# terran-project/terran

Hardware: AMD Instinct MI355X
Metric: frames/sec 1080p detect+embed+pose (higher is better)
Workload: dtype f16x3: operands x = hi + lo (two IEEE halfs, 22 bits), 3 f16 MFMAs per product, f32 accumulate; float32-grade results; 1 GPU; BASELINE configs[4]: 1080p detect+embed+pose; Detection(short_side=416) + Recognition(top-2) + Estimation(short_side=184); 32 frames per GPU per step resident in HBM; random-init weights; precision=f16x3, frames_per_gpu_step=32, faces_per_frame=2, resident_batch_reused=True, batches_in_flight_per_gpu=2

## Files before the change

### terran_amd/build.py

```python
import os
import subprocess
import sys

HERE = os.path.dirname(os.path.abspath(__file__))
CSRC = os.path.join(HERE, 'csrc')
LIB = os.path.join(HERE, 'libterran_amd.so')
SOURCES = ['runtime.hip', 'conv_split.hip', 'conv_split_modes.hip', 'conv_sym.hip', 'conv_dwpw.hip', 'conv_igemm.hip', 'layers.hip', 'net.hip', 'retinaface_post.hip', 'arcface_post.hip',
           'openpose_post.hip', 'draw.hip', 'jpeg_host.hip', 'jpeg.hip',
           'jpeg_encode.hip']
FLAGS = ['--offload-arch=gfx950', '-O3', '-std=c++17', '-fPIC', '-Wall', '-Wno-unused-function']


STAMP = LIB + '.stamp'


def source_hash():
    import hashlib
    h = hashlib.sha256(' '.join(FLAGS).encode())
    files = [os.path.join(CSRC, f) for f in sorted(os.listdir(CSRC)) if f.endswith(('.hip', '.h'))]
    files.append(os.path.join(os.path.dirname(HERE), 'include', 'terran_amd.h'))
    for f in files:
        with open(f, 'rb') as fh:
            h.update(os.path.basename(f).encode() + b'\0' + fh.read())
    return h.hexdigest()


def _stale(target, deps):
    if not os.path.exists(target):
        return True
    t = os.path.getmtime(target)
    return any(os.path.getmtime(d) > t for d in deps)


def _unit_hash(src, headers, flags):
    import hashlib
    h = hashlib.sha256(' '.join(flags).encode())
    for f in [src] + sorted(headers):
        with open(f, 'rb') as fh:
            h.update(os.path.basename(f).encode() + b'\0' + fh.read())
    return h.hexdigest()


def build(force=False, verbose=False):
    hipcc = os.environ.get('HIPCC', '/opt/rocm/bin/hipcc')
    headers = [os.path.join(CSRC, f) for f in os.listdir(CSRC) if f.endswith('.h')]
    headers.append(os.path.join(os.path.dirname(HERE), 'include', 'terran_amd.h'))
    extra_all = os.environ.get('TA_EXTRA_FLAGS', '').split()
    objs = []
    procs = []
    for src in SOURCES:
        s = os.path.join(CSRC, src)
        if not os.path.exists(s):
            continue
        o = os.path.join(CSRC, src.replace('.hip', '.o'))
        objs.append(o)
        exact = src.endswith('_post.hip') or src == 'draw.hip'
        flags = FLAGS + (['-ffp-contract=off'] if exact else []) + extra_all
        want = _unit_hash(s, headers, flags)
        try:
            with open(o + '.stamp') as fh:
# ... 88 lines not shown
```

### terran_amd/csrc/net.hip

```cpp
#include <stdlib.h>
#include <string.h>

#include <algorithm>
#include <chrono>

#include "act_format.h"
#include "ta_internal.h"

static int conv_out(int in, int k, int stride, int pad) { return (in + 2 * pad - k) / stride + 1; }

static bool conv_ksplit_eligible(const ta_op_desc& op, int in_fmt) {
  const int kblk = in_fmt == TA_FMT_F16 ? 64 : 32;
  const bool uniform = (op.cin % kblk == 0) && (op.n_slabs == op.kh * op.kw * (op.cin / kblk));
  const bool kernel_ok = in_fmt == ta_split_fmt_of(op.prec);
  return uniform && kernel_ok && op.groups <= 1 && !op.pool;
}

#define TA_MAX_PLANS 4
#define TA_MAX_PLAN_BYTES ((size_t)96 << 30)

static void destroy_plan(ta_plan* pl) {
  if (!pl) return;
  if (pl->arena) (void)hipFree(pl->arena);
  if (pl->ktab_dev) (void)hipFree(pl->ktab_dev);
// ... 232 lines not shown
static const float* wptr(const ta_model* m, int64_t off) { return off < 0 ? nullptr : (const float*)(m->weights_dev + off); }

static void print_op_profile(ta_model* m, std::vector<hipEvent_t>& ev) {
  (void)hipStreamSynchronize(m->ctx->stream);
  double tot_ms = 0, tot_fl = 0;
  for (size_t oi = 0; oi < m->ops.size(); ++oi) {
    const ta_op_desc& op = m->ops[oi];
    const ta_tensor& to = m->tensors[op.out];
    float ms = 0.f;
    (void)hipEventElapsedTime(&ms, ev[2 * oi], ev[2 * oi + 1]);
    const ta_tensor& ti = m->tensors[op.in];
    const double M = op.type == TA_OP_CONV && op.pool
                         ? (double)m->run_n * conv_out(ti.h, op.kh, op.stride, op.pad) * conv_out(ti.w, op.kw, op.stride, op.pad)
                         : (double)m->run_n * to.h * to.w;
    const double fl = (op.type == TA_OP_CONV || op.type == TA_OP_DWPW) ? 2.0 * op.macs_per_pixel * M : 0.0;
    tot_ms += ms;
    tot_fl += fl;
    fprintf(stderr, "op %3zu type %d k%dx%d s%d g%d cin %4d cout %4d  %3dx%-3d M %8.0f slabs %4d  %8.1f us %7.1f TF\n", oi, op.type, op.kh,
            op.kw, op.stride, op.groups, op.cin, op.cout, to.h, to.w, M, op.n_slabs, ms * 1e3, ms > 0 ? fl / (ms * 1e-3) / 1e12 : 0.0);
  }
  fprintf(stderr, "model kind %d n %d: %.3f ms in ops, %.1f GFLOP, %.1f TF\n", m->kind, m->run_n, tot_ms, tot_fl / 1e9, tot_fl / (tot_ms * 1e-3) / 1e12);
  for (auto e : ev) (void)hipEventDestroy(e);
}

int ta_model_run_ops(ta_model* m) {
  ta_ctx* ctx = m->ctx;
  static const bool prof_ops = getenv("TA_PROFILE_OPS") != nullptr;
  std::vector<hipEvent_t> ev;
  if (prof_ops) {
    ev.resize(2 * m->ops.size());
    for (auto& e : ev) (void)hipEventCreate(&e);
  }
  struct fin_t {
    ta_model* m;
    std::vector<hipEvent_t>& ev;
    bool on;
    ~fin_t() { if (on) print_op_profile(m, ev); }
  } fin{m, ev, prof_ops};
  static const bool no_lanes = getenv("TA_NO_LANES") != nullptr;
  const bool lanes_on = !prof_ops && !ctx->profiling && !no_lanes;
  struct lanes_t {
    ta_ctx* ctx;
    hipStream_t main;
    bool started[2] = {false, false};
    ~lanes_t() {
      ctx->stream = main;
      for (int i = 0; i < 2; ++i)
        if (started[i]) {
          (void)hipEventRecord(ctx->side_join[i], ctx->side_stream[i]);
          (void)hipStreamWaitEvent(main, ctx->side_join[i], 0);
        }
    }
  } lanes{ctx, ctx->stream};
  for (size_t oi = 0; oi < m->ops.size(); ++oi) {
    const ta_op_desc& op = m->ops[oi];
    const ta_tensor& ti = m->tensors[op.in];
    const ta_tensor& to = m->tensors[op.out];
    const int lane = lanes_on ? (op.variant >> 17) & 3 : 0;
    ctx->stream = lanes.main;
    if (lane) {
      const int li = lane - 1;
      if (!ctx->side_stream[li]) {
        TA_HIP(ctx, hipStreamCreateWithFlags(&ctx->side_stream[li], hipStreamNonBlocking));
        TA_HIP(ctx, hipEventCreateWithFlags(&ctx->side_fork[li], hipEventDisableTiming));
        TA_HIP(ctx, hipEventCreateWithFlags(&ctx->side_join[li], hipEventDisableTiming));
      }
      if (!lanes.started[li]) {
        TA_HIP(ctx, hipEventRecord(ctx->side_fork[li], lanes.main));
        TA_HIP(ctx, hipStreamWaitEvent(ctx->side_stream[li], ctx->side_fork[li], 0));
        lanes.started[li] = true;
      }
      ctx->stream = ctx->side_stream[li];
    }
    struct evp_t {
      hipEvent_t e;
      hipStream_t s;
      bool on;
      ~evp_t() { if (on) (void)hipEventRecord(e, s); }
    } evp{prof_ops ? ev[2 * oi + 1] : nullptr, ctx->stream, prof_ops};
    if (prof_ops) (void)hipEventRecord(ev[2 * oi], ctx->stream);
    switch (op.type) {
      case TA_OP_CONV: {
        ta_conv_launch p;
        memset(&p, 0, sizeof(p));
        p.in = ti.dev;
        p.w = wptr(m, op.w_off);
        p.ktab = m->ktab_dev + m->ktab_off[oi];
        p.bias = wptr(m, op.bias_off);
        p.prelu = wptr(m, op.prelu_off);
        p.out = to.dev;
        p.M = m->run_n * to.h * to.w;
        p.Ho = to.h;
        p.Wo = to.w;
        p.n_slabs = op.n_slabs;
        p.coutp = op.coutp;
        p.cout = op.cout;
        p.act = op.act;
        p.stride = op.stride;
        p.prec = op.prec;
        const int kblk = ti.fmt == TA_FMT_F16 ? 64 : 32;
        p.uniform_k = (op.cin % kblk == 0) && (op.n_slabs == op.kh * op.kw * (op.cin / kblk));
        p.k_cblocks = op.cin / kblk;
        if (ti.fmt == TA_FMT_F16 && (!p.uniform_k || op.in_ch_off || op.groups > 1 || op.prec != 4))
          return ta_fail(ctx, TA_E_INVALID, "op %zu: a half-float tensor feeds whole-tensor convs of the f16 mode only", oi);
        p.k_w = op.kw;
        p.k_h = op.kh;
// ... 2 lines not shown
        p.in_row = ti.wp() * ti.cf();
        p.in_pix = ti.cf();
        p.win_wp = ti.wp();
        p.win_img = ti.hp() * ti.wp();
        p.in_off0 = (int)(((size_t)(ti.halo - op.pad) * ti.wp() + (ti.halo - op.pad)) * ti.cf());
        p.out_img = (int)((size_t)to.hp() * to.wp() * to.cf());
        p.out_row = to.wp() * to.cf();
        p.out_pix = to.cf();
        p.out_off0 = (int)to.off(0, 0, 0);
        p.out_ch = op.out_ch_off;
        p.out_fmt = to.fmt;
        p.in_fmt = ti.fmt;
        if (op.res >= 0) {
          const ta_tensor& tr = m->tensors[op.res];
          p.res = tr.dev;
          p.res_img = (int)((size_t)tr.hp() * tr.wp() * tr.cf());
          p.res_row = tr.wp() * tr.cf();
          p.res_pix = tr.cf();
          p.res_off0 = (int)tr.off(0, 0, 0);
          p.res_ch = op.res_ch_off;
          p.res_fmt = tr.fmt;
          p.res_up2 = op.res_up2;
        }
        if (op.out2 >= 0) {
          const ta_tensor& t2 = m->tensors[op.out2];
          p.out2 = t2.dev;
          p.scale2 = wptr(m, op.scale2_off);
          p.shift2 = wptr(m, op.shift2_off);
          p.o2_img = (int)((size_t)t2.hp() * t2.wp() * t2.cf());
          p.o2_row = t2.wp() * t2.cf();
          p.o2_pix = t2.cf();
          p.o2_off0 = (int)t2.off(0, 0, 0);
          p.o2_ch = op.out2_ch_off;
          p.o2_fmt = t2.fmt;
        }
        if (op.groups > 1) {
          p.group_cout = op.cout / op.groups;
          p.group_cin = op.cin;
        }
        p.variant = op.variant & 255;
        if ((op.variant >> 16) & 1) p.bias9 = wptr(m, op.scale2_off);
        p.range_check = (m->has_half_ops && (m->tensor_read[op.out] || (op.out2 >= 0 && m->tensor_read[op.out2]))) ? 1 : 0;
        p.amax_index = (m->amax_on && oi < TA_AMAX_OPS) ? (int)oi : -1;
        double flops = 2.0 * op.macs_per_pixel * (double)p.M;
        if (op.pool) {
          p.pool = 1;
          p.M = m->run_n * to.h * to.w * 4;
          flops = 2.0 * op.macs_per_pixel * (double)m->run_n * conv_out(ti.h, op.kh, op.stride, op.pad) *
                  conv_out(ti.w, op.kw, op.stride, op.pad);
        }
        p.k_split = m->splitk_ws ? ta_conv_ksplit(p.coutp, p.n_slabs, conv_ksplit_eligible(op, ti.fmt), (op.variant >> 8) & 255) : 1;
        p.partial = m->splitk_ws;
        if (lane) p.k_split = 1;
        TA_TRY(ta_launch_conv(ctx, p, flops));
        break;
      }
      case TA_OP_RFSTEM:
        TA_TRY(ta_launch_rfstem(ctx, m->input_u8, m->run_n, ti.h, ti.w, (const float*)m->weights_host_small.data(),
                                op.cout == 32 ? wptr(m, op.w_off) + 448 : nullptr, to));
        break;
      case TA_OP_DWPW: {
        ta_conv_launch p;
        memset(&p, 0, sizeof(p));
        p.in = ti.dev;
        p.w = wptr(m, op.w_off);
        p.bias = wptr(m, op.bias_off);
        p.dw_w = wptr(m, op.scale2_off);
        p.dw_bias = wptr(m, op.shift2_off);
        p.dw_c = op.cin;
        p.dw_stride = op.stride;
        p.out = to.dev;
        p.M = m->run_n * to.h * to.w;
        p.Ho = to.h;
        p.Wo = to.w;
        p.n_slabs = op.n_slabs;
        p.coutp = op.coutp;
        p.cout = op.cout;
        p.act = op.act;
        p.stride = 1;
        p.prec = op.prec;
        p.range_check = (m->has_half_ops && m->tensor_read[op.out]) ? 1 : 0;
        p.amax_index = (m->amax_on && oi < TA_AMAX_OPS) ? (int)oi : -1;
        p.in_img = (int)((size_t)ti.hp() * ti.wp() * ti.c);
        p.in_row = ti.wp() * ti.c;
        p.in_pix = ti.c;
        p.in_off0 = (int)(((size_t)(ti.halo - 1) * ti.wp() + (ti.halo - 1)) * ti.c);
        p.in_fmt = ti.fmt;
        p.out_img = (int)((size_t)to.hp() * to.wp() * to.c);
        p.out_row = to.wp() * to.c;
        p.out_pix = to.c;
        p.out_off0 = (int)to.off(0, 0, 0);
        p.out_ch = op.out_ch_off;
        p.out_fmt = to.fmt;
        TA_TRY(ta_launch_dwpw(ctx, p, 2.0 * op.macs_per_pixel * (double)p.M));
        break;
      }
      case TA_OP_DWCONV: {
        ta_dw_launch p;
        memset(&p, 0, sizeof(p));
        p.in = ti.dev;
        p.w = wptr(m, op.w_off);
        p.bias = wptr(m, op.bias_off);
        p.out = to.dev;
        p.N = m->run_n;
        p.Ho = to.h;
        p.Wo = to.w;
// ... 349 lines not shown
```

### terran_amd/csrc/ta_internal.h

```cpp
#pragma once
#include <hip/hip_runtime.h>
#include <stdint.h>
#include <stdio.h>
#include <atomic>
#include <map>
#include <mutex>
#include <string>
#include <vector>

#include "../../include/terran_amd.h"

#define TA_BLOB_MAGIC 0x314D4154u

enum {
  TA_OP_CONV = 1,
  TA_OP_DWCONV = 2,
  TA_OP_MAXPOOL = 3,
  TA_OP_COPYCH = 4,
  TA_OP_RFSTEM = 5,
  TA_OP_DWPW = 6
};
enum { TA_ACT_NONE = 0, TA_ACT_RELU = 1, TA_ACT_PRELU = 2 };

struct ta_blob_header {
// ... 201 lines not shown
struct ta_conv_launch {
  const float* in;
  const float* w;
  const int32_t* ktab;
  const float* bias;
  const float* prelu;
  float* out;
  const float* res;
  float* out2;
  const float* scale2;
  const float* shift2;
  int M, Ho, Wo, n_slabs, coutp, cout, act, stride, prec;
  int uniform_k, k_cblocks, k_w, k_h, in_ch_off;
  int in_img, in_row, in_pix, in_off0;
  int out_img, out_row, out_pix, out_off0, out_ch, out_fmt;
  int res_img, res_row, res_pix, res_off0, res_up2, res_ch, res_fmt;
  int o2_img, o2_row, o2_pix, o2_off0, o2_ch, o2_fmt;
  int in_fmt;
  int win_wp, win_img;
  int group_cout, group_cin;
  int k_split;
  float* partial;
  int variant;
  const float* dw_w;
  const float* dw_bias;
  int dw_c, dw_stride;
  int pool;
  float r_nct, r_tile_blocks, r_Wo, r_Ho, r_HoWo;
  int fast_div;
  int fast_drain;
#ifdef TA_CONV_TRACE
  int trace_block;
#endif
  const float* bias9;
  int range_check;
  int amax_index;
  int* range_flag;
};

static inline int ta_split_fmt_of(int prec) { return prec == 0 ? 0  : (prec == 4 ? 3  : ((prec == 3 || prec == 5) ? 2  : 1 )); }

static inline int ta_conv_ksplit(int coutp, int n_slabs, bool eligible, int packed = 0) {
  if (!eligible || coutp % 128) return 1;
  if (packed > 1) return packed <= n_slabs ? packed : 1;
  if (n_slabs < 512) return 1;
  return 32;
}

int ta_launch_conv(ta_ctx* ctx, const ta_conv_launch& p, double flops);
int ta_launch_conv_sym(ta_ctx* ctx, int variant, const ta_conv_launch& p);
int ta_launch_conv_split(ta_ctx* ctx, int variant, const ta_conv_launch& p);
int ta_launch_conv_split_modes(ta_ctx* ctx, int variant, const ta_conv_launch& p);
int ta_launch_dwpw(ta_ctx* ctx, const ta_conv_launch& p, double flops);
int ta_win_patch_rows(const ta_conv_launch& p, int BM);
#define TA_WIN_PR_2x2 384
#define TA_WIN_PR_2x4 448
#define TA_WIN_PR_1x4 512
struct ta_frames;
int ta_launch_rfstem(ta_ctx* ctx, const uint8_t* frames_dev, int n, int h, int w, const float* weights_host, const float* w2_dev, const struct ta_tensor& out);

struct ta_dw_launch {
  const float* in;
  const float* w;
  const float* bias;
  float* out;
  int N, Ho, Wo, C, stride, relu;
  int in_img, in_row, in_pix, in_off0, in_fmt;
  int out_img, out_row, out_pix, out_off0, out_fmt;
};
int ta_launch_dwconv(ta_ctx* ctx, const ta_dw_launch& p);
int ta_launch_maxpool(ta_ctx* ctx, const ta_tensor& in, const ta_tensor& out, int n);
int ta_launch_copych(ta_ctx* ctx, const ta_tensor& in, int in_ch, const ta_tensor& out, int out_ch, int ch, int n);

enum { TA_PRE_RETINAFACE = 1, TA_PRE_OPENPOSE = 2, TA_PRE_ARCFACE_CROPS = 3 };
int ta_launch_preprocess(ta_ctx* ctx, int mode, const uint8_t* src_dev, int n, int h, int w, const ta_tensor& dst);

struct ta_plan {
  int n = 0, h = 0, w = 0;
  std::vector<ta_tensor> tensors;
  char* arena = nullptr;
  size_t arena_bytes = 0;
  int32_t* ktab_dev = nullptr;
  std::vector<size_t> ktab_off;
  float* splitk_ws = nullptr;
  uint64_t last_use = 0;
};

struct ta_model {
  ta_ctx* ctx = nullptr;
  int kind = 0;
  ta_blob_header hdr;
  std::vector<ta_tensor_desc> tdesc;
  std::vector<ta_op_desc> ops;
  char* weights_dev = nullptr;
  bool has_half_ops = false;
  bool amax_on = false;
  std::vector<char> tensor_read;
  std::vector<std::vector<float>> unscale_host;
  std::vector<char> weights_host_small;
  std::vector<ta_plan*> plans;
  ta_plan* active = nullptr;
  uint64_t use_counter = 0;
  int plan_n = 0, plan_h = 0, plan_w = 0;
  int run_n = 0;
  const uint8_t* input_u8 = nullptr;
  std::vector<ta_tensor> tensors;
// ... 8 lines not shown
```

### terran_amd/pack.py

```python
import os

import numpy as np

from . import arch

MODEL_RETINAFACE, MODEL_ARCFACE, MODEL_OPENPOSE = 1, 2, 3
OP_CONV, OP_DWCONV, OP_MAXPOOL, OP_COPYCH, OP_RFSTEM, OP_DWPW = 1, 2, 3, 4, 5, 6
ACT_NONE, ACT_RELU, ACT_PRELU = 0, 1, 2
MAGIC = 0x314D4154

HEADER_DT = np.dtype({
    'names': ['magic', 'version', 'kind', 'n_tensors', 'n_ops', 'input_tensor', 'n_outputs', 'outputs',
              'tensors_off', 'ops_off', 'weights_off', 'weights_bytes'],
    'formats': ['<u4', '<u4', '<i4', '<i4', '<i4', '<i4', '<i4', ('<i4', 16), '<i8', '<i8', '<i8', '<i8'],
    'offsets': [0, 4, 8, 12, 16, 20, 24, 28, 96, 104, 112, 120],
    'itemsize': 128,
})
TENSOR_DT = np.dtype([('channels', '<i4'), ('halo', '<i4'), ('alias_of', '<i4'), ('fmt', '<i4'), ('unscale_off', '<i4')])
FMT_F32, FMT_SPLIT, FMT_SPLIT16, FMT_F16 = 0, 1, 2, 3
_OP_I32 = ['type', 'in', 'out', 'in_ch_off', 'cin', 'out_ch_off', 'cout', 'coutp', 'kh', 'kw', 'stride', 'pad',
           'act', 'res', 'res_ch_off', 'res_up2', 'out2', 'out2_ch_off', 'n_slabs', 'prec', 'groups', 'variant', 'pool', 'wscale_log2']
_OP_I64 = ['w_off', 'bias_off', 'prelu_off', 'scale2_off', 'shift2_off', 'wus_off']
OP_DT = np.dtype([(n, '<i4') for n in _OP_I32] + [(n, '<i8') for n in _OP_I64] + [('macs_per_pixel', '<f8')])
assert OP_DT.itemsize == 152 and TENSOR_DT.itemsize == 20
BLOB_VERSION = 9


PACK_SWITCHES = ('TERRAN_AMD_NO_FUSED_POOL', 'TERRAN_AMD_NO_GROUPED', 'TERRAN_AMD_NO_MERGED_OUTPUTS', 'TERRAN_AMD_ARCFACE_SECOND_OUTPUT',
                 'TERRAN_AMD_NO_STAGE4_KSPLIT', 'TERRAN_AMD_DETECTOR_F32', 'TERRAN_AMD_DETECTOR_BASE_F32', 'TERRAN_AMD_NO_FUSED_DETECTOR', 'TERRAN_AMD_NO_FUSED_FRONT',
                 'TERRAN_AMD_NO_DETECTOR_LANES', 'TERRAN_AMD_NO_ACT_SCALES')


def active_switches():
    return tuple((k, os.environ[k]) for k in PACK_SWITCHES if os.environ.get(k))


_SOURCE_TAG = []


def source_tag():
    if not _SOURCE_TAG:
        import hashlib
        h = hashlib.sha256()
        here = os.path.dirname(os.path.abspath(__file__))
        try:
            for f in ('pack.py', 'arch.py'):
                with open(os.path.join(here, f), 'rb') as fh:
                    h.update(fh.read())
            _SOURCE_TAG.append(h.hexdigest()[:10])
        except OSError:
            _SOURCE_TAG.append(None)
    return _SOURCE_TAG[0]


PRECISIONS = {'f32': 0, 'bf16x3': 1, 'bf16': 2, 'f16x3': 3, 'f16': 4, 'f16x2': 5}
SPLIT_FMT = {0: FMT_F32, 1: FMT_SPLIT, 2: FMT_SPLIT, 3: FMT_SPLIT16, 4: FMT_F16, 5: FMT_SPLIT16}


def _rup(x, m):
    return (x + m - 1) // m * m


def _bf16_bits(x):
    u = np.ascontiguousarray(x, dtype=np.float32).view(np.uint32)
    return ((u + np.uint32(0x7FFF) + ((u >> np.uint32(16)) & np.uint32(1))) >> np.uint32(16)).astype(np.uint16)


def _bf16_to_f32(b):
    return (b.astype(np.uint32) << np.uint32(16)).view(np.float32)


def split_bf16_rows(packed):
    hi = _bf16_bits(packed)
    lo = _bf16_bits(packed - _bf16_to_f32(hi))
    rows = np.concatenate([hi, lo], axis=-1)
    return np.ascontiguousarray(rows).view(np.float32)


def row_exponents(packed):
    m = np.abs(np.asarray(packed, np.float32)).max(axis=(0, 2)).astype(np.float64)
    ok = np.isfinite(m) & (m > 0)
    s = np.zeros(m.shape, np.int64)
    s[ok] = np.clip(13 - np.floor(np.log2(m[ok])), -60, 60).astype(np.int64)
# ... 134 lines not shown
            if tid == self.input_tensor:
                self.stats[tid][2][:] = True
        return self.stats[tid]

    def _write_stats(self, tid, ch_off, mu, var, amax=None):
        st = self._stats_of(tid)
        n = len(mu)
        if amax is None:
            amax = np.abs(mu) + _ACT_SIGMAS * np.sqrt(var)
        new = ~st[2][ch_off:ch_off + n]
        take = new | (amax > st[3][ch_off:ch_off + n])
        st[0][ch_off:ch_off + n][take] = mu[take]
        st[1][ch_off:ch_off + n][take] = var[take]
        st[3][ch_off:ch_off + n] = np.where(new, amax, np.maximum(amax, st[3][ch_off:ch_off + n]))
        st[2][ch_off:ch_off + n] = True

    @staticmethod
    def _act_bound(mu, var, act, slope=None):
        sd = np.sqrt(np.maximum(var, 0.0))
        hi, lo = mu + _ACT_SIGMAS * sd, _ACT_SIGMAS * sd - mu
        if act == ACT_NONE:
            return np.maximum(hi, lo)
        if act == ACT_RELU or slope is None:
            return np.maximum(hi, 4.0 * sd)
        a = np.abs(np.asarray(slope, np.float64))
        return np.maximum(np.maximum(hi, a * lo), 4.0 * sd * np.maximum(a, 1.0))

    @staticmethod
    def _conv_moments(full, bias, mu_in, var_in, groups, cout):
        taps, cin_p, coutp = full.shape
        f64 = full.astype(np.float64)
        wsum = f64.sum(0)
        wsq = (f64 * f64).sum(0)
        rho = _TAP_CORR if taps > 1 else 0.0
        wvar = (1.0 - rho) * wsq + rho * wsum * wsum
        mu = np.zeros(coutp)
        var = np.zeros(coutp)
        if groups > 1:
            cg = cout // groups
            for g in range(groups):
                sl = slice(g * cg, (g + 1) * cg)
                mu[sl] = mu_in[g * cin_p:(g + 1) * cin_p] @ wsum[:, sl]
                var[sl] = var_in[g * cin_p:(g + 1) * cin_p] @ wvar[:, sl]
        else:
            mu = mu_in[:cin_p] @ wsum
            var = var_in[:cin_p] @ wvar
        b = np.zeros(coutp)
        if bias is not None:
            b[:cout] = np.asarray(bias, np.float64)
        return (mu + b)[:cout], np.maximum(var[:cout], 0.0)

    def conv(self, tin, tout, W, bias, *, stride=1, pad=None, act=ACT_NONE, in_ch_off=0, ch_pos=None, cin_p=None,
             out_ch_off=0, cout_p=None, prelu=None, res=-1, res_ch_off=0, res_up2=0, out2=-1, out2_ch_off=0,
             scale2=None, shift2=None, groups=1, variant=0, pool=False, k_split=0, precision=None, in_affine=None):
        W = np.asarray(W, dtype=np.float64)
        cout, cin, kh, kw = W.shape
        bias9 = None
        if in_affine is not None:
            assert (kh, kw, stride) == (3, 3, 1) and pad in (None, 1) and groups == 1 and out2 < 0 and scale2 is None and not pool
            W, bias9 = fold_input_affine(W, bias, *in_affine)
            bias = bias9[5]
        if groups > 1:
            assert cout % groups == 0 and cin % 32 == 0 and (cout // groups) % 128 == 0 and ch_pos is None
        if pad is None:
            pad = kh // 2
        if pool:
            assert groups == 1 and res < 0 and out2 < 0 and stride == 1 and cin % 32 == 0 and cout % 64 == 0 and ch_pos is None
        if cin_p is None:
            cin_p = _rup(cin, 4)
        if ch_pos is None:
            ch_pos = np.arange(cin)
        if cout_p is None:
            cout_p = _rup(cout, 4)
        coutp = _rup(cout_p, 32)
        K = kh * kw * cin_p
        n_slabs = _rup(K, 32) // 32
        full = np.zeros((kh * kw, cin_p, coutp), np.float32)
        full[:, np.asarray(ch_pos), :cout] = W.transpose(2, 3, 1, 0).reshape(kh * kw, cin, cout)
        flat = np.zeros((n_slabs * 32, coutp), np.float32)
        flat[:K] = full.reshape(K, coutp)
        prec = self.prec if precision is None else PRECISIONS[precision]

        def vec(v, fill=0.0):
            if v is None:
                return -1, None
            out = np.full(coutp, fill, np.float64)
            out[:cout] = np.asarray(v, dtype=np.float64)
            return self._w(out), out
        fold = dict(flat=flat, taps=kh * kw, cin_p=cin_p, K=K)
        scale2_off = -1
        if bias9 is not None:
            t9 = np.zeros((16, coutp), np.float64)
            t9[:, :cout] = bias9
            scale2_off = self._w(t9)
            fold['bias9'] = t9
            variant |= 1 << 16
        else:
            scale2_off, fold['scale2'] = vec(scale2)
        bvec = np.zeros(coutp, np.float64)
        if bias is not None:
            bvec[:cout] = np.asarray(bias, np.float64)
        fold['bias'] = bvec
        bias_off = self._w(np.concatenate([bvec, np.ones(coutp)]))
        wus_off = bias_off + 4 * coutp
        prelu_off, _ = vec(prelu)
        shift2_off, fold['shift2'] = vec(shift2)
        op = dict(type=OP_CONV, out=tout, in_ch_off=in_ch_off, cin=cin_p, out_ch_off=out_ch_off, cout=cout_p,
                  coutp=coutp, kh=kh, kw=kw, stride=stride, pad=pad, act=act, res=res, res_ch_off=res_ch_off,
                  res_up2=res_up2, out2=out2, out2_ch_off=out2_ch_off, n_slabs=n_slabs, prec=prec,
                  groups=groups, variant=variant | (int(k_split) << 8) | (self.lane << 17), pool=int(bool(pool)), wscale_log2=0,
                  w_off=self._w_reserve(n_slabs * coutp * 128), bias_off=bias_off, prelu_off=prelu_off, scale2_off=scale2_off,
                  shift2_off=shift2_off, wus_off=wus_off, macs_per_pixel=float(cout * cin * kh * kw))
        op['in'] = tin
        self._fold[len(self.ops)] = fold
        self.ops.append(op)
        st_in = self._stats_of(tin)
        span = cin_p * max(groups, 1)
        mu, var = self._conv_moments(full, bias, st_in[0][in_ch_off:in_ch_off + span], st_in[1][in_ch_off:in_ch_off + span],
                                     groups, cout)
        slope = None if prelu is None else np.asarray(prelu, np.float64)
        bound = self._act_bound(mu, var, act, slope)
        mu, var = act_moments(mu, var, act, slope)
        if res >= 0:
            st_r = self._stats_of(res)
            mu = mu + st_r[0][res_ch_off:res_ch_off + cout]
            var = var + st_r[1][res_ch_off:res_ch_off + cout]
            bound = bound + st_r[3][res_ch_off:res_ch_off + cout]
        if pool:
            mu, var = mu + 1.03 * np.sqrt(var), 0.49 * var
        self._write_stats(tout, out_ch_off, mu, var, bound)
        if out2 >= 0:
            s2, h2 = np.asarray(scale2, np.float64), np.asarray(shift2, np.float64)
            self._write_stats(out2, out2_ch_off, mu * s2 + h2, var * s2 * s2, np.abs(s2) * bound + np.abs(h2))

    def dwconv(self, tin, tout, W, bias, *, stride=1, relu=True):
        C = W.shape[0]
        w9 = np.asarray(W, dtype=np.float64).reshape(C, 9).T
        op = dict(type=OP_DWCONV, out=tout, in_ch_off=0, cin=C, out_ch_off=0, cout=C, coutp=_rup(C, 32), kh=3,
                  kw=3, stride=stride, pad=1, act=ACT_RELU if relu else ACT_NONE, res=-1, res_ch_off=0, res_up2=0,
                  out2=-1, out2_ch_off=0, n_slabs=0, prec=0, groups=1, variant=0, pool=0, wscale_log2=0, w_off=self._w(w9), bias_off=self._w(bias),
                  prelu_off=-1, scale2_off=-1, shift2_off=-1, wus_off=-1, macs_per_pixel=float(C * 9))
        op['in'] = tin
        self.ops.append(op)
        st = self._stats_of(tin)
        mu, var = self._dw_moments(w9, bias, st[0][:C], st[1][:C])
        act = ACT_RELU if relu else ACT_NONE
        self._write_stats(tout, 0, *act_moments(mu, var, act), self._act_bound(mu, var, act))

    @staticmethod
    def _dw_moments(w9, bias, mu_in, var_in):
        w9 = np.asarray(w9, np.float64)
        wsum, wsq = w9.sum(0), (w9 * w9).sum(0)
        return (np.asarray(bias, np.float64) + mu_in * wsum,
                var_in * ((1.0 - _TAP_CORR) * wsq + _TAP_CORR * wsum * wsum))

    def rfstem(self, tin, tout, Ws, bs, Wd, bd, Wp, bp, Wd2=None, bd2=None, Wp2=None, bp2=None):
        parts = [np.asarray(Ws, np.float64).reshape(8, 27).ravel(), np.asarray(bs, np.float64),
                 np.asarray(Wd, np.float64).reshape(8, 9).T.ravel(), np.asarray(bd, np.float64),
                 np.asarray(Wp, np.float64).reshape(16, 8).ravel(), np.asarray(bp, np.float64)]
        fuse = Wd2 is not None
        if fuse:
            parts += [np.asarray(Wd2, np.float64).reshape(16, 9).T.ravel(), np.asarray(bd2, np.float64),
                      np.asarray(Wp2, np.float64).reshape(32, 16).T.ravel(), np.asarray(bp2, np.float64)]
# ... 313 lines not shown
                    parts[8] = (parts[8].reshape(16, 32) * up[None, :32]).ravel()
                    parts[9] = parts[9] * up[:32]
                else:
                    parts[4] = (parts[4].reshape(16, 8) * up[:16, None]).ravel()
                    parts[5] = parts[5] * up[:16]
                self._rewrite(op['w_off'], np.concatenate(parts))
        ops = np.zeros(len(self.ops), OP_DT)
        for i, op in enumerate(self.ops):
            for k, v in op.items():
                ops[i][k] = v
        t_off = HEADER_DT.itemsize
        o_off = t_off + tens.nbytes
        w_off = _rup(o_off + ops.nbytes, 256)
        outs = np.full(16, -1, np.int32)
        outs[:len(self.outputs)] = self.outputs
        hdr[0] = (MAGIC, BLOB_VERSION, self.kind, len(self.tensors), len(self.ops), self.input_tensor, len(self.outputs), outs,
                  t_off, o_off, w_off, self.wbytes)
        head = hdr.tobytes() + tens.tobytes() + ops.tobytes()
        for f in self._fold.values():
            f.pop('flat', None)
        self._blob = head + b'\0' * (w_off - len(head)) + b''.join(self.wchunks)
        return self._blob


def _bn_affine(sd, key, eps):
    g = np.asarray(sd[key + '.weight'], np.float64)
    b = np.asarray(sd[key + '.bias'], np.float64)
    m = np.asarray(sd[key + '.running_mean'], np.float64)
    v = np.asarray(sd[key + '.running_var'], np.float64)
    s = g / np.sqrt(v + eps)
    return s, b - m * s


def _fold(W, bias, scale, shift):
    W = np.asarray(W, np.float64) * scale[:, None, None, None]
    b0 = np.zeros(W.shape[0]) if bias is None else np.asarray(bias, np.float64)
    return W, b0 * scale + shift


OP_FEAT, OP_PAF, OP_HM, OP_XCH = 0, 128, 168, 192


def pack_openpose(sd, precision='f32'):
    if precision in ('f16', 'f16x2'):
        precision = 'f16x3'
    P = Program(MODEL_OPENPOSE, precision)
    t = P.tensor(4, 1, name='input')
    P.input_tensor = t
    P.input_stats = (np.array([-0.05, -0.05, -0.05, 0.0]), np.array([0.08, 0.08, 0.08, 0.0]))
    X0 = P.tensor(OP_XCH, 3, name='X0')
    X1 = P.tensor(OP_XCH, 3, name='X1')
    items = arch.OPENPOSE_MODEL0
    fuse_pool = not os.environ.get('TERRAN_AMD_NO_FUSED_POOL')
    skip_pool = False
    for i, item in enumerate(items):
        nxt = items[i + 1] if i + 1 < len(items) else None
        if item[0] == 'pool':
            if skip_pool:
                skip_pool = False
                continue
            o = P.tensor(P.tensors[t][0], 1)
            P.simple(OP_MAXPOOL, t, o)
            t = o
            continue
        name, cin, cout, k = item
        W, b = sd['model0.%s.weight' % name], sd['model0.%s.bias' % name]
        if nxt is None:
            P.conv(t, X0, W, b, act=ACT_RELU, out_ch_off=OP_FEAT)
            P.tap('feat', X0, OP_FEAT, 128)
        elif nxt[0] == 'pool' and fuse_pool and cin % 32 == 0 and cout % 64 == 0:
            o = P.tensor(cout, 1, name=name + '_pooled')
            P.conv(t, o, W, b, act=ACT_RELU, pool=True)
            t = o
            skip_pool = True
        else:
            o = P.tensor(cout, 0 if nxt[0] == 'pool' else 1, name=name)
            P.conv(t, o, W, b, act=ACT_RELU)
            t = o
    P.simple(OP_COPYCH, X0, X1, OP_FEAT, OP_FEAT, 128)

    cat_pos = np.concatenate([OP_PAF + np.arange(38), OP_HM + np.arange(19), OP_FEAT + np.arange(128)])
    for st in range(1, 7):
        xin, xout = (X0, X1) if st % 2 == 1 else (X1, X0)
        l1, l2 = arch.openpose_stage_layers(st, 1), arch.openpose_stage_layers(st, 2)
        (n1, cin, c1, k, r1), (n2, cin2, c2, k2, r2) = l1[0], l2[0]
        assert (cin, k, r1) == (cin2, k2, r2) and c1 == c2 == 128
        W = np.concatenate([np.asarray(sd['model%d_%d.%s.weight' % (st, br, n)]) for br, n in ((1, n1), (2, n2))])
        b = np.concatenate([np.asarray(sd['model%d_%d.%s.bias' % (st, br, n)]) for br, n in ((1, n1), (2, n2))])
        kw = dict(ch_pos=cat_pos, cin_p=OP_XCH) if cin == 185 else dict(in_ch_off=OP_FEAT)
        cur = P.tensor(c1 + c2, l1[1][3] // 2)
        P.conv(xin, cur, W, b, act=ACT_RELU if r1 else ACT_NONE, **kw)
        grouped = not os.environ.get('TERRAN_AMD_NO_GROUPED')
        for li in range(1, len(l1) - 1):
            (na, cin, cout, k, relu), (nb, cin2, cout2, k2, relu2) = l1[li], l2[li]
            if not grouped:
                o = P.tensor(2 * cout, l1[li + 1][3] // 2)
                for br, n in ((1, na), (2, nb)):
                    key = 'model%d_%d.%s' % (st, br, n)
                    P.conv(cur, o, sd[key + '.weight'], sd[key + '.bias'], act=ACT_RELU if relu else ACT_NONE,
                           in_ch_off=(br - 1) * cin, out_ch_off=(br - 1) * cout)
                cur = o
                continue
            assert (cin, cout, k, relu) == (cin2, cout2, k2, relu2) and cin % 32 == 0 and cout % 128 == 0
            W = np.concatenate([np.asarray(sd['model%d_%d.%s.weight' % (st, br, n)]) for br, n in ((1, na), (2, nb))])
            b = np.concatenate([np.asarray(sd['model%d_%d.%s.bias' % (st, br, n)]) for br, n in ((1, na), (2, nb))])
            o = P.tensor(2 * cout, l1[li + 1][3] // 2)
            P.conv(cur, o, W, b, act=ACT_RELU if relu else ACT_NONE, groups=2)
            cur = o
        (np_, cin, co1, k, r1), (nh, cin2, co2, k2, r2) = l1[-1], l2[-1]
        if r1 == r2 and cin == cin2 <= 128 and not os.environ.get('TERRAN_AMD_NO_MERGED_OUTPUTS'):
            Wp, bp = np.asarray(sd['model%d_1.%s.weight' % (st, np_)]), np.asarray(sd['model%d_1.%s.bias' % (st, np_)])
            Wh, bh = np.asarray(sd['model%d_2.%s.weight' % (st, nh)]), np.asarray(sd['model%d_2.%s.bias' % (st, nh)])
            Wm = np.zeros((60, 2 * cin, 1, 1), np.float32)
            bm = np.zeros(60, np.float32)
            Wm[0:co1, :cin], bm[0:co1] = Wp, bp
            Wm[40:40 + co2, cin:], bm[40:40 + co2] = Wh, bh
            P.conv(cur, xout, Wm, bm, act=ACT_RELU if r1 else ACT_NONE, out_ch_off=OP_PAF, cout_p=60)
            P.ops[-1]['macs_per_pixel'] = float((co1 + co2) * cin)
        else:
            for br, layers in ((1, l1), (2, l2)):
                name, cin, cout, k, relu = layers[-1]
                key = 'model%d_%d.%s' % (st, br, name)
                off, cp = (OP_PAF, 40) if br == 1 else (OP_HM, 20)
                P.conv(cur, xout, sd[key + '.weight'], sd[key + '.bias'], act=ACT_RELU if relu else ACT_NONE,
                       in_ch_off=(br - 1) * cin, out_ch_off=off, cout_p=cp)
        P.tap('stage%d_paf' % st, xout, OP_PAF, 38)
        P.tap('stage%d_hm' % st, xout, OP_HM, 19)
    P.outputs = [X0]
    P.tap('pafs', X0, OP_PAF, 38)
    P.tap('heatmaps', X0, OP_HM, 19)
# ... 209 lines not shown
```

Measured before the change: 2234 frames/s.

## Fuse OpenPose stem conv1+conv2+pool into one kernel

Adds a dedicated kernel that computes the first 3x3 conv (3->64) of the pose network for an 8x32 tile plus halo directly into LDS, then runs the second 3x3 conv with fused ReLU and 2x2 max-pool. The first conv's full-resolution activation is never written to HBM. The runtime holds the first conv launch and, when the next op qualifies, launches the fused kernel in place of both convs. This removes a large intermediate write/read and one launch, at the cost of recomputing halo pixels and a large LDS footprint that limits occupancy.

```diff
diff --git a/terran_amd/build.py b/terran_amd/build.py
--- a/terran_amd/build.py
+++ b/terran_amd/build.py
@@ -5,7 +5,7 @@
 HERE = os.path.dirname(os.path.abspath(__file__))
 CSRC = os.path.join(HERE, 'csrc')
 LIB = os.path.join(HERE, 'libterran_amd.so')
-SOURCES = ['runtime.hip', 'conv_split.hip', 'conv_split_modes.hip', 'conv_sym.hip', 'conv_dwpw.hip', 'conv_igemm.hip', 'layers.hip', 'net.hip', 'retinaface_post.hip', 'arcface_post.hip',
+SOURCES = ['runtime.hip', 'conv_split.hip', 'conv_split_modes.hip', 'conv_sym.hip', 'conv_dwpw.hip', 'conv_stem.hip', 'conv_igemm.hip', 'layers.hip', 'net.hip', 'retinaface_post.hip', 'arcface_post.hip',
            'openpose_post.hip', 'draw.hip', 'jpeg_host.hip', 'jpeg.hip',
            'jpeg_encode.hip']
 FLAGS = ['--offload-arch=gfx950', '-O3', '-std=c++17', '-fPIC', '-Wall', '-Wno-unused-function']
diff --git a/terran_amd/csrc/conv_stem.hip b/terran_amd/csrc/conv_stem.hip
--- /dev/null
+++ b/terran_amd/csrc/conv_stem.hip
@@ -0,0 +1,342 @@
+#include <string.h>
+
+#include "conv_split_kernels.h"
+
+constexpr int ST_TH = 8, ST_TW = 32;
+constexpr int ST_PW = ST_TW + 2, ST_PH = ST_TH + 2;
+constexpr int ST_NPATCH = ST_PW * ST_PH;
+constexpr int ST_PR = 352;
+constexpr int ST_IW = ST_TW + 4, ST_IH = ST_TH + 4;
+constexpr int ST_NIN = ST_IW * ST_IH;
+constexpr int ST_S = 18;
+constexpr int ST_A_STAGE = 64 * 32;
+constexpr int ST_PATCH = ST_PR * 32;
+constexpr size_t ST_LDS_BYTES = (size_t)(3 * ST_A_STAGE + 2 * ST_PATCH + 2 * 64 * 32 + ST_NIN * 4) * sizeof(float);
+static_assert(ST_NPATCH <= ST_PR && ST_PR % 32 == 0, "patch rows");
+static_assert((size_t)256 * 64 * 4 <= (size_t)(3 * ST_A_STAGE + 2 * ST_PATCH) * 4, "the parked tile fits the ring + patches");
+static_assert(ST_LDS_BYTES <= 160 * 1024, "one workgroup's LDS");
+
+struct ta_stem_args {
+  const float* in;
+  const float* w1;
+  const float* bias1;
+  const float* w2;
+  const float* bias2;
+  float* out;
+  int* range_flag;
+  int H, W, Hp, Wp;
+  int tiles_x, tiles_y, n_tiles;
+  int in_img, in_row, in_halo;
+  int out_img, out_row, out_pix, out_off0, out_ch;
+  int range_check1, amax1, amax2;
+};
+
+__device__ __forceinline__ void stem_range_report(const ta_stem_args& p, unsigned amax, int slot) {
+  if (amax > TA_F16_MAX_BITS) *p.range_flag = 1;
+  if (slot >= 0 && amax) atomicMax((unsigned*)p.range_flag + TA_AMAX_SLOT0 + 2 * slot, amax);
+}
+
+__global__ __launch_bounds__(512, 2) void pose_stem_kernel(const ta_stem_args p) {
+  constexpr int PREC = PREC_F16X3;
+  constexpr int NC = 4, NP = 4, BN = 64;
+  constexpr int QA = BN / 8 / NP;
+  extern __shared__ __attribute__((aligned(16))) float lds[];
+  float* const patch0 = lds + 3 * ST_A_STAGE;
+  float* const w1s = patch0 + 2 * ST_PATCH;
+  float* const in_s = w1s + 2 * 64 * 32;
+
+  const int tid = threadIdx.x;
+  const int lane = tid & 63;
+  const int wave = __builtin_amdgcn_readfirstlane(tid >> 6);
+  const int tile = ta_xcd_tile(p.n_tiles, blockIdx.x & 7, blockIdx.x >> 3);
+  if (tile < 0) return;
+  const int per_img = p.tiles_x * p.tiles_y;
+  const int img = tile / per_img;
+  const int trem = tile - img * per_img;
+  const int tyi = trem / p.tiles_x, txi = trem - tyi * p.tiles_x;
+  const int Y0 = tyi * ST_TH, X0 = txi * ST_TW;
+
+  const int pw = wave - NC;
+  const int lchunk = (lane & 7) ^ ((4 * (pw & 1) + (lane >> 4)) & 7);
+  unsigned a_off[QA];
+#pragma unroll
+  for (int q = 0; q < QA; ++q) a_off[q] = (unsigned)((((q * NP + pw) * 8 + (lane >> 3)) * 32 + lchunk * 4) * 4);
+  int gi = 0;
+  auto issue_a = [&](int stage) {
+    const int a_slab = gi < 9 ? 2 * gi : 2 * (gi - 9) + 1;
+#pragma unroll
+    for (int q = 0; q < QA; ++q) ta_dma16((const char*)p.w2 + (size_t)a_slab * (BN * 128), a_off[q], lds + stage * ST_A_STAGE + (q * NP + pw) * 256);
+    ++gi;
+  };
+  if (wave >= NC) {
+    issue_a(0);
+    issue_a(1);
+  }
+
+  for (int i = tid; i < 2 * 64 * 8; i += 512) {
+    const int row = i >> 3, c = i & 7;
+    *(f32x4*)(w1s + row * 32 + ((c ^ ((row >> 1) & 7)) << 2)) = *(const f32x4*)(p.w1 + row * 32 + c * 4);
+  }
+  if (tid < ST_NIN) {
+    const int iy = tid / ST_IW, ix = tid - iy * ST_IW;
+    const int y = Y0 - 2 + iy, x = X0 - 2 + ix;
+    f32x4 v = {0.f, 0.f, 0.f, 0.f};
+    if (y >= -p.in_halo && y < p.H + p.in_halo && x >= -p.in_halo && x < p.W + p.in_halo)
+      v = *(const f32x4*)(p.in + (size_t)img * p.in_img + (size_t)(y + p.in_halo) * p.in_row + (size_t)(x + p.in_halo) * 4);
+    *(f32x4*)(in_s + tid * 4) = v;
+  }
+  __syncthreads();
+  const int frow = lane & 31;
+  const int fsw = (frow >> 1) & 7;
+  const int kg = lane >> 5;
+  {
+    unsigned amax = 0;
+    for (int g = wave; g < ST_PR / 32; g += NC + NP) {
+      const int pr = g * 32 + frow;
+      const int prc = pr < ST_NPATCH ? pr : 0;
+      const int py = prc / ST_PW, px = prc - py * ST_PW;
+      f32x16 acc[2];
+#pragma unroll
+      for (int a = 0; a < 2; ++a)
+#pragma unroll
+        for (int r = 0; r < 16; ++r) acc[a][r] = 0.f;
+#pragma unroll
+      for (int s = 0; s < 2; ++s)
+#pragma unroll
+        for (int t = 0; t < 2; ++t) {
+          bf16x8 ah[2], al[2], bh, bl;
+#pragma unroll
+          for (int a = 0; a < 2; ++a) {
+            ah[a] = *(const bf16x8*)(w1s + (s * 64 + a * 32 + frow) * 32 + ((2 * kg + t) ^ fsw) * 4);
+            al[a] = *(const bf16x8*)(w1s + (s * 64 + a * 32 + frow) * 32 + ((4 + 2 * kg + t) ^ fsw) * 4);
+          }
+          f32x4 x[2];
+#pragma unroll
+          for (int h = 0; h < 2; ++h) {
+            const int q = s * 8 + 4 * kg + 2 * t + h;
+            const int tap = q < 9 ? q : 0;
+            const int ky = (tap * 11) >> 5, kx = tap - 3 * ky;
+            x[h] = *(const f32x4*)(in_s + ((py + ky) * ST_IW + px + kx) * 4);
+          }
+#pragma unroll
+          for (int e = 0; e < 4; ++e) {
+            const __bf16 h0 = ta_to16<PREC>(x[0][e]), h1 = ta_to16<PREC>(x[1][e]);
+            bh[e] = h0;
+            bh[4 + e] = h1;
+            bl[e] = ta_to16<PREC>(x[0][e] - ta_from16<PREC>(h0));
+            bl[4 + e] = ta_to16<PREC>(x[1][e] - ta_from16<PREC>(h1));
+          }
+#pragma unroll
+          for (int a = 0; a < 2; ++a) acc[a] = ta_mfma16<PREC>(al[a], bh, acc[a]);
+#pragma unroll
+          for (int a = 0; a < 2; ++a) acc[a] = ta_mfma16<PREC>(ah[a], bl, acc[a]);
+#pragma unroll
+          for (int a = 0; a < 2; ++a) acc[a] = ta_mfma16<PREC>(ah[a], bh, acc[a]);
+        }
+      const int oy = Y0 - 1 + py, ox = X0 - 1 + px;
+      const bool inmap = pr < ST_NPATCH && oy >= 0 && oy < p.H && ox >= 0 && ox < p.W;
+      const int sw = (pr >> 1) & 7;
+#pragma unroll
+      for (int a = 0; a < 2; ++a) {
+        char* const row = (char*)(patch0 + a * ST_PATCH) + pr * 128;
+#pragma unroll
+        for (int j = 0; j < 4; ++j) {
+          const int co = a * 32 + 8 * j + 4 * kg;
+          const f32x4 b4 = *(const f32x4*)(p.bias1 + co), u4 = *(const f32x4*)(p.bias1 + 64 + co);
+          f32x4 v;
+#pragma unroll
+          for (int e = 0; e < 4; ++e) v[e] = inmap ? ta_relu(__builtin_fmaf(acc[a][4 * j + e], u4[e], b4[e])) : 0.f;
+          if (p.range_check1) amax = ta_amax4(amax, v);
+          unsigned h0, h1, l0, l1;
+          ta_pack2<true>(v[0], v[1], h0, l0);
+          ta_pack2<true>(v[2], v[3], h1, l1);
+          *(uint2*)(row + ((j ^ sw) << 4) + 8 * kg) = make_uint2(h0, h1);
+          *(uint2*)(row + (((4 + j) ^ sw) << 4) + 8 * kg) = make_uint2(l0, l1);
+        }
+      }
+    }
+    stem_range_report(p, amax, p.amax1);
+  }
+  asm volatile("s_waitcnt vmcnt(0)" ::: "memory");
+  __syncthreads();
+
+  if (wave >= NC) {
+    int stage = 2;
+    for (int g = 0; g < ST_S; ++g) {
+      if (g + 1 < ST_S) asm volatile("s_waitcnt vmcnt(%0)" ::"n"(QA) : "memory");
+      else asm volatile("s_waitcnt vmcnt(0)" ::: "memory");
+      __builtin_amdgcn_s_barrier();
+      asm volatile("" ::: "memory");
+      if (g + 2 < ST_S) {
+        issue_a(stage);
+        stage = stage == 2 ? 0 : stage + 1;
+      }
+    }
+    __builtin_amdgcn_s_barrier();
+    __builtin_amdgcn_s_barrier();
+    asm volatile("" ::: "memory");
+  } else {
+    const int cn = wave;
+    f32x16 acc[2][2];
+    split_acc_clear(acc);
+    const int a_row0 = frow;
+    int rB[2];
+#pragma unroll
+    for (int b = 0; b < 2; ++b) rB[b] = (cn * 2 + b) * ST_PW + frow;
+    struct Frag {
+      bf16x8 ah[2], al[2], bh[2], bl[2];
+    };
+    unsigned pb[2];
+    auto baddr = [&](int tap_off, int buf) {
+#pragma unroll
+      for (int b = 0; b < 2; ++b) {
+        const unsigned row = (unsigned)(rB[b] + tap_off);
+        pb[b] = (unsigned)buf * (unsigned)(ST_PATCH * 4) + row * 128u + ((((unsigned)(2 * kg)) ^ ((row >> 1) & 7u)) << 4);
+      }
+    };
+    auto load = [&](Frag& f, const float* st, int t) {
+#pragma unroll
+      for (int a = 0; a < 2; ++a) {
+        f.ah[a] = *(const bf16x8*)(st + (a_row0 + a * 32) * 32 + ((2 * kg + t) ^ fsw) * 4);
+        f.al[a] = *(const bf16x8*)(st + (a_row0 + a * 32) * 32 + ((4 + 2 * kg + t) ^ fsw) * 4);
+      }
+#pragma unroll
+      for (int b = 0; b < 2; ++b) {
+        f.bh[b] = *(const bf16x8*)((const char*)patch0 + (pb[b] ^ (unsigned)(t << 4)));
+        f.bl[b] = *(const bf16x8*)((const char*)patch0 + ((pb[b] ^ (unsigned)(t << 4)) ^ 64u));
+      }
+    };
+    auto mma = [&](const Frag& f) { split_mma16<PREC>(acc, f.ah, f.al, f.bh, f.bl); };
+    int kx = 0, ky = 0, cb = 0, tap_off = 0, stage = 0;
+    Frag F0, F1;
+    baddr(0, 0);
+    __builtin_amdgcn_s_barrier();
+    asm volatile("" ::: "memory");
+    load(F0, lds, 0);
+    for (int g = 0; g + 1 < ST_S; ++g) {
+      const float* st = lds + stage * ST_A_STAGE;
+      stage = stage == 2 ? 0 : stage + 1;
+      __builtin_amdgcn_sched_barrier(0);
+      load(F1, st, 1);
+      mma(F0);
+      split_pin<8, 12>();
+      __builtin_amdgcn_sched_barrier(0);
+      if (++kx == 3) {
+        kx = 0;
+        tap_off += ST_PW - 3;
+        if (++ky == 3) {
+          ky = 0;
+          ++cb;
+          tap_off = -1;
+        }
+      }
+      ++tap_off;
+      asm volatile("s_waitcnt lgkmcnt(0)" ::: "memory");
+      baddr(tap_off, cb);
+      __builtin_amdgcn_s_barrier();
+      asm volatile("" ::: "memory");
+      load(F0, lds + stage * ST_A_STAGE, 0);
+      mma(F1);
+      split_pin<8, 12>();
+      __builtin_amdgcn_sched_barrier(0);
+    }
+    load(F1, lds + stage * ST_A_STAGE, 1);
+    mma(F0);
+    mma(F1);
+    __builtin_amdgcn_s_barrier();
+    asm volatile("" ::: "memory");
+    conv_epilogue_park<BN>(acc, lds, 0, cn, lane);
+    asm volatile("s_waitcnt lgkmcnt(0)" ::: "memory");
+    __builtin_amdgcn_s_barrier();
+    asm volatile("" ::: "memory");
+  }
+
+  {
+    constexpr int NCH = BN / 4;
+    const int k8 = tid & 7, w = tid >> 3;
+    const int wy = w >> 4, wx = w & 15;
+    const int co = 8 * k8;
+    float bias[8], us[8];
+    *(f32x4*)bias = *(const f32x4*)(p.bias2 + co);
+    *(f32x4*)(bias + 4) = *(const f32x4*)(p.bias2 + co + 4);
+    *(f32x4*)us = *(const f32x4*)(p.bias2 + 64 + co);
+    *(f32x4*)(us + 4) = *(const f32x4*)(p.bias2 + 64 + co + 4);
+    float r[4][8];
+#pragma unroll
+    for (int i = 0; i < 4; ++i) {
+      const int row = (2 * wy + (i >> 1)) * ST_TW + 2 * wx + (i & 1);
+      const int sw = row & (NCH - 1);
+      *(f32x4*)r[i] = *(const f32x4*)(lds + (row * NCH + ((2 * k8) ^ sw)) * 4);
+      *(f32x4*)(r[i] + 4) = *(const f32x4*)(lds + (row * NCH + ((2 * k8 + 1) ^ sw)) * 4);
+#pragma unroll
+      for (int e = 0; e < 8; ++e) r[i][e] = ta_relu(__builtin_fmaf(r[i][e], us[e], bias[e]));
+    }
+    float v[8];
+#pragma unroll
+    for (int e = 0; e < 8; ++e) v[e] = fmaxf(fmaxf(r[0][e], r[1][e]), fmaxf(r[2][e], r[3][e]));
+    const int qy = tyi * (ST_TH / 2) + wy, qx = txi * (ST_TW / 2) + wx;
+    unsigned amax = 0;
+    if (qy < p.Hp && qx < p.Wp) {
+      char* const ob = (char*)p.out + ta_split_chan(p.out_ch + co);
+      ta_split_store8<1>(ob + 4u * (unsigned)(img * p.out_img + qy * p.out_row + qx * p.out_pix + p.out_off0), v, amax);
+    }
+    stem_range_report(p, amax, p.amax2);
+  }
+}
+
+bool ta_pose_stem_eligible(const ta_ctx* ctx, const ta_conv_launch& c1, const ta_conv_launch& c2) {
+  if (ctx->conv_force || c1.variant || c2.variant) return false;
+  const bool first = c1.prec == PREC_F16X3 && c1.in_fmt == TA_FMT_F32 && c1.in_pix == 4 && c1.in_ch_off == 0 && c1.k_w == 3 && c1.k_h == 3 &&
+                     c1.stride == 1 && c1.n_slabs == 2 && c1.coutp == 64 && c1.cout == 64 && c1.act == TA_ACT_RELU && !c1.res && !c1.out2 &&
+                     !c1.bias9 && !c1.pool && !c1.group_cout && c1.out_fmt == TA_FMT_SPLIT16 && c1.out_ch == 0;
+  const bool second = c2.prec == PREC_F16X3 && c2.in_fmt == TA_FMT_SPLIT16 && c2.in == c1.out && c2.in_ch_off == 0 && c2.uniform_k &&
+                      c2.k_cblocks == 2 && c2.k_w == 3 && c2.k_h == 3 && c2.stride == 1 && c2.n_slabs == ST_S && c2.coutp == 64 && c2.cout == 64 &&
+                      c2.act == TA_ACT_RELU && c2.pool == 1 && !c2.res && !c2.out2 && !c2.bias9 && !c2.group_cout &&
+                      c2.out_fmt == TA_FMT_SPLIT16 && (c2.out_ch & 7) == 0;
+  if (!first || !second) return false;
+  if (c1.Ho < 46 || c1.Wo < 81 || c2.Ho != c1.Ho / 2 || c2.Wo != c1.Wo / 2 || c2.Ho <= 0 || c2.Wo <= 0) return false;
+  if (c1.M % (c1.Ho * c1.Wo) || c2.M != 4 * (c1.M / (c1.Ho * c1.Wo)) * c2.Ho * c2.Wo) return false;
+  const long long n = c1.M / (c1.Ho * c1.Wo);
+  if (((n + 1) * c2.out_img + c2.out_off0) * 4 >= (1LL << 32)) return false;
+  return (long long)n * ((c2.Ho + 3) / 4) * ((c2.Wo + 15) / 16) < (1LL << 28);
+}
+
+int ta_launch_pose_stem(ta_ctx* ctx, const ta_conv_launch& c1, const ta_conv_launch& c2, double flops) {
+  ta_stem_args a;
+  memset(&a, 0, sizeof(a));
+  const int n = c1.M / (c1.Ho * c1.Wo);
+  if (n <= 0) return TA_OK;
+  a.in = c1.in;
+  a.w1 = c1.w;
+  a.bias1 = c1.bias;
+  a.w2 = c2.w;
+  a.bias2 = c2.bias;
+  a.out = c2.out;
+  a.range_flag = ctx->range_flag;
+  a.H = c1.Ho;
+  a.W = c1.Wo;
+  a.Hp = c2.Ho;
+  a.Wp = c2.Wo;
+  a.tiles_y = (a.Hp + ST_TH / 2 - 1) / (ST_TH / 2);
+  a.tiles_x = (a.Wp + ST_TW / 2 - 1) / (ST_TW / 2);
+  a.n_tiles = n * a.tiles_y * a.tiles_x;
+  a.in_img = c1.in_img;
+  a.in_row = c1.in_row;
+  a.in_halo = (c1.win_wp - c1.Wo) / 2;
+  a.out_img = c2.out_img;
+  a.out_row = c2.out_row;
+  a.out_pix = c2.out_pix;
+  a.out_off0 = c2.out_off0;
+  a.out_ch = c2.out_ch;
+  a.range_check1 = c1.range_check;
+  a.amax1 = c1.amax_index;
+  a.amax2 = c2.amax_index;
+  if (a.in_halo < 1) return ta_fail(ctx, TA_E_INVALID, "pose front: the input tensor has no halo");
+  ctx->cur_flops = flops;
+  ta_prof_scope scope(ctx, 0, flops);
+  TA_SET_LDS_ATTR(ctx, pose_stem_kernel, ST_LDS_BYTES);
+  TA_NOTE_KERNEL(ctx, "pose_stem_kernel");
+  hipLaunchKernelGGL(pose_stem_kernel, dim3(((a.n_tiles + 7) / 8) * 8), dim3(512), ST_LDS_BYTES, ctx->stream, a);
+  TA_HIP(ctx, hipGetLastError());
+  return TA_OK;
+}
diff --git a/terran_amd/csrc/net.hip b/terran_amd/csrc/net.hip
--- a/terran_amd/csrc/net.hip
+++ b/terran_amd/csrc/net.hip
@@ -308,6 +308,9 @@
         }
     }
   } lanes{ctx, ctx->stream};
+  ta_conv_launch stem_p;
+  double stem_flops = 0;
+  bool stem_held = false;
   for (size_t oi = 0; oi < m->ops.size(); ++oi) {
     const ta_op_desc& op = m->ops[oi];
     const ta_tensor& ti = m->tensors[op.in];
@@ -416,6 +419,22 @@
         p.k_split = m->splitk_ws ? ta_conv_ksplit(p.coutp, p.n_slabs, conv_ksplit_eligible(op, ti.fmt), (op.variant >> 8) & 255) : 1;
         p.partial = m->splitk_ws;
         if (lane) p.k_split = 1;
+        if (stem_held) {
+          stem_held = false;
+          if (ta_pose_stem_eligible(ctx, stem_p, p)) {
+            TA_TRY(ta_launch_pose_stem(ctx, stem_p, p, stem_flops + flops));
+            break;
+          }
+          TA_TRY(ta_launch_conv(ctx, stem_p, stem_flops));
+        } else if (((op.variant >> 19) & 1) && !lane && op.pad == 1 && oi + 1 < m->ops.size()) {
+          const ta_op_desc& nx = m->ops[oi + 1];
+          if (nx.type == TA_OP_CONV && nx.in == op.out && nx.pad == 1 && !((nx.variant >> 17) & 3)) {
+            stem_p = p;
+            stem_flops = flops;
+            stem_held = true;
+            break;
+          }
+        }
         TA_TRY(ta_launch_conv(ctx, p, flops));
         break;
       }
diff --git a/terran_amd/csrc/ta_internal.h b/terran_amd/csrc/ta_internal.h
--- a/terran_amd/csrc/ta_internal.h
+++ b/terran_amd/csrc/ta_internal.h
@@ -277,6 +277,8 @@
 int ta_launch_conv_split(ta_ctx* ctx, int variant, const ta_conv_launch& p);
 int ta_launch_conv_split_modes(ta_ctx* ctx, int variant, const ta_conv_launch& p);
 int ta_launch_dwpw(ta_ctx* ctx, const ta_conv_launch& p, double flops);
+bool ta_pose_stem_eligible(const ta_ctx* ctx, const ta_conv_launch& c1, const ta_conv_launch& c2);
+int ta_launch_pose_stem(ta_ctx* ctx, const ta_conv_launch& c1, const ta_conv_launch& c2, double flops);
 int ta_win_patch_rows(const ta_conv_launch& p, int BM);
 #define TA_WIN_PR_2x2 384
 #define TA_WIN_PR_2x4 448
diff --git a/terran_amd/pack.py b/terran_amd/pack.py
--- a/terran_amd/pack.py
+++ b/terran_amd/pack.py
@@ -28,7 +28,7 @@
 
 PACK_SWITCHES = ('TERRAN_AMD_NO_FUSED_POOL', 'TERRAN_AMD_NO_GROUPED', 'TERRAN_AMD_NO_MERGED_OUTPUTS', 'TERRAN_AMD_ARCFACE_SECOND_OUTPUT',
                  'TERRAN_AMD_NO_STAGE4_KSPLIT', 'TERRAN_AMD_DETECTOR_F32', 'TERRAN_AMD_DETECTOR_BASE_F32', 'TERRAN_AMD_NO_FUSED_DETECTOR', 'TERRAN_AMD_NO_FUSED_FRONT',
-                 'TERRAN_AMD_NO_DETECTOR_LANES', 'TERRAN_AMD_NO_ACT_SCALES')
+                 'TERRAN_AMD_NO_DETECTOR_LANES', 'TERRAN_AMD_NO_ACT_SCALES', 'TERRAN_AMD_NO_FUSED_STEM')
 
 
 def active_switches():
@@ -269,7 +269,7 @@
 
     def conv(self, tin, tout, W, bias, *, stride=1, pad=None, act=ACT_NONE, in_ch_off=0, ch_pos=None, cin_p=None,
              out_ch_off=0, cout_p=None, prelu=None, res=-1, res_ch_off=0, res_up2=0, out2=-1, out2_ch_off=0,
-             scale2=None, shift2=None, groups=1, variant=0, pool=False, k_split=0, precision=None, in_affine=None):
+             scale2=None, shift2=None, groups=1, variant=0, pool=False, k_split=0, precision=None, in_affine=None, fuse_next=False):
         W = np.asarray(W, dtype=np.float64)
         cout, cin, kh, kw = W.shape
         bias9 = None
@@ -325,7 +325,7 @@
         op = dict(type=OP_CONV, out=tout, in_ch_off=in_ch_off, cin=cin_p, out_ch_off=out_ch_off, cout=cout_p,
                   coutp=coutp, kh=kh, kw=kw, stride=stride, pad=pad, act=act, res=res, res_ch_off=res_ch_off,
                   res_up2=res_up2, out2=out2, out2_ch_off=out2_ch_off, n_slabs=n_slabs, prec=prec,
-                  groups=groups, variant=variant | (int(k_split) << 8) | (self.lane << 17), pool=int(bool(pool)), wscale_log2=0,
+                  groups=groups, variant=variant | (int(k_split) << 8) | (self.lane << 17) | (int(bool(fuse_next)) << 19), pool=int(bool(pool)), wscale_log2=0,
                   w_off=self._w_reserve(n_slabs * coutp * 128), bias_off=bias_off, prelu_off=prelu_off, scale2_off=scale2_off,
                   shift2_off=shift2_off, wus_off=wus_off, macs_per_pixel=float(cout * cin * kh * kw))
         op['in'] = tin
@@ -745,6 +745,7 @@
     X1 = P.tensor(OP_XCH, 3, name='X1')
     items = arch.OPENPOSE_MODEL0
     fuse_pool = not os.environ.get('TERRAN_AMD_NO_FUSED_POOL')
+    fuse_stem = P.prec == PRECISIONS['f16x3'] and not os.environ.get('TERRAN_AMD_NO_FUSED_STEM')
     skip_pool = False
     for i, item in enumerate(items):
         nxt = items[i + 1] if i + 1 < len(items) else None
@@ -768,7 +769,7 @@
             skip_pool = True
         else:
             o = P.tensor(cout, 0 if nxt[0] == 'pool' else 1, name=name)
-            P.conv(t, o, W, b, act=ACT_RELU)
+            P.conv(t, o, W, b, act=ACT_RELU, fuse_next=fuse_stem and i == 0 and cin == 3 and fuse_pool)
             t = o
     P.simple(OP_COPYCH, X0, X1, OP_FEAT, OP_FEAT, 128)
 
```

Result: slower. 2145 frames/s (-4.0%).
